# gcorso/DiffDock

Measured on AMD Instinct MI355X. Metric: poses/sec (20 steps x 40 samples, DiffDock-L score model), higher is better.
Workload: dtype f32

## Files before the change

diffdock_amd/csrc/api.cpp:

```cpp
#include <cstdlib>
#include <cstring>

#include "model.h"

using namespace ddmi;

struct ddmi_model { Model m; };

static thread_local std::string g_err;

template <class F> static int guard(F&& f) {
  try { f(); return DDMI_OK; }
  catch (const Error& e) { g_err = e.what(); return e.code; }
  catch (const std::exception& e) { g_err = e.what(); return DDMI_ERR_ARG; }
}

Routes ddmi::resolve_routes(const ddmi_config& cfg, int n_cus) {
  static const struct { const char* name; int32_t ddmi_exec_options::*field; int max; } ranges[] = {
      {"streams", &ddmi_exec_options::streams, 1}, {"dense_rows", &ddmi_exec_options::dense_rows, 2},
      {"shared_tiles", &ddmi_exec_options::shared_tiles, 2}, {"packed_granules", &ddmi_exec_options::packed_granules, 1},
      {"merged_granule", &ddmi_exec_options::merged_granule, 1}, {"pre_reduce", &ddmi_exec_options::pre_reduce, 1},
      {"hidden_mm", &ddmi_exec_options::hidden_mm, 1}, {"fc1_batch", &ddmi_exec_options::fc1_batch, 1},
      {"tile_split", &ddmi_exec_options::tile_split, 8}, {"tile_split_small", &ddmi_exec_options::tile_split_small, 8},
      {"hidden_grid", &ddmi_exec_options::hidden_grid, 1 << 20}, {"tp_apply", &ddmi_exec_options::tp_apply, 3},
// ... 178 lines not shown
    DDMI_REQUIRE(h && lig_pos && tr && rot, DDMI_ERR_ARG, "null argument");
    DDMI_CHECK_HIP(hipSetDevice(h->m.device));
    modify_conformer(h->m, lig_pos, tr, rot, tor, (hipStream_t)s);
  });
}

int ddmi_sample(ddmi_model* h, float* lig_pos, const ddmi_sample_cfg* cfg, ddmi_stream s) {
  return guard([&] {
    DDMI_REQUIRE(h && lig_pos && cfg, DDMI_ERR_ARG, "null argument");
    DDMI_CHECK_HIP(hipSetDevice(h->m.device));
    sample(h->m, lig_pos, *cfg, (hipStream_t)s);
  });
}

int ddmi_set_sample_record(ddmi_model* h, const ddmi_sample_record* r) {
  return guard([&] {
    DDMI_REQUIRE(h, DDMI_ERR_ARG, "null model");
    set_sample_record(h->m, r);
  });
}

int ddmi_perturb(ddmi_model* h, float* tr, float* rot, float* tor, const ddmi_sample_cfg* cfg, int step, ddmi_stream s) {
  return guard([&] {
    DDMI_REQUIRE(h && tr && rot && cfg, DDMI_ERR_ARG, "null argument");
    DDMI_CHECK_HIP(hipSetDevice(h->m.device));
    perturb(h->m, tr, rot, tor, *cfg, step, (hipStream_t)s);
  });
}

int ddmi_debug_shape(ddmi_model* h, const char* name, int64_t shape[4], int* ndim, int* is_int) {
  return guard([&] {
    DDMI_REQUIRE(h && name, DDMI_ERR_ARG, "null argument");
    auto it = h->m.debug.find(name);
    DDMI_REQUIRE(it != h->m.debug.end(), DDMI_ERR_KEY, std::string("unknown debug buffer: ") + name);
    *ndim = (int)it->second.shape.size();
    for (int d = 0; d < *ndim && d < 4; ++d) shape[d] = it->second.shape[d];
    *is_int = it->second.is_int;
  });
}

int ddmi_debug_read(ddmi_model* h, const char* name, void* dst, size_t bytes, ddmi_stream s) {
  return guard([&] {
    DDMI_REQUIRE(h && name && dst, DDMI_ERR_ARG, "null argument");
    auto it = h->m.debug.find(name);
    DDMI_REQUIRE(it != h->m.debug.end(), DDMI_ERR_KEY, std::string("unknown debug buffer: ") + name);
    size_t n = 4;
    for (auto d : it->second.shape) n *= (size_t)d;
    DDMI_REQUIRE(bytes <= n, DDMI_ERR_ARG, "read past the end of the buffer");
    DDMI_CHECK_HIP(hipStreamSynchronize((hipStream_t)s));
    DDMI_CHECK_HIP(hipMemcpy(dst, it->second.ptr, bytes, hipMemcpyDeviceToHost));
  });
}

int ddmi_wigner_3j(int l1, int l2, int l3, double* out) {
  return guard([&] {
    DDMI_REQUIRE(out && l1 >= 0 && l2 >= 0 && l3 >= std::abs(l1 - l2) && l3 <= l1 + l2, DDMI_ERR_ARG, "bad l");
    auto w = wigner_3j(l1, l2, l3);
    std::memcpy(out, w.data(), w.size() * sizeof(double));
  });
}

int ddmi_debug_philox(const uint32_t* counters, const uint32_t* keys, int n, uint32_t* host_out) {
  return guard([&] {
    DDMI_REQUIRE(counters && keys && host_out && n > 0, DDMI_ERR_ARG, "null argument");
    struct Buf {
      unsigned* p = nullptr;
      explicit Buf(size_t bytes) { DDMI_CHECK_HIP(hipMalloc(reinterpret_cast<void**>(&p), bytes)); }
      ~Buf() { if (p) (void)hipFree(p); }
    };
    Buf c((size_t)n * 16), k((size_t)n * 8), o((size_t)n * 16);
    hipStream_t st = nullptr;
    DDMI_CHECK_HIP(hipStreamCreateWithFlags(&st, hipStreamNonBlocking));
    struct StreamGuard { hipStream_t s; ~StreamGuard() { (void)hipStreamDestroy(s); } } sg{st};
    DDMI_CHECK_HIP(hipMemcpyAsync(c.p, counters, (size_t)n * 16, hipMemcpyHostToDevice, st));
    DDMI_CHECK_HIP(hipMemcpyAsync(k.p, keys, (size_t)n * 8, hipMemcpyHostToDevice, st));
    launch_debug_philox(c.p, k.p, n, o.p, st);
    DDMI_CHECK_HIP(hipMemcpyAsync(host_out, o.p, (size_t)n * 16, hipMemcpyDeviceToHost, st));
    DDMI_CHECK_HIP(hipStreamSynchronize(st));
// ... 32 lines not shown
```

diffdock_amd/csrc/conv_layers.cpp:

```cpp
#include <cmath>
#include <cstdio>
#include <numeric>
#include <string>

#include "cx.h"

namespace ddmi {
namespace {

long tiles_of(const RunGroup& q) {
  const long gn = std::max(1, q.gcount);
  return std::max(1L, gn * (((long)q.ea_rows / gn + 31) / 32) / 16);
}
constexpr long CHIP_TILES = 256;
bool chip_filling(long tiles) { return tiles >= CHIP_TILES; }

bool vn_fresh(const Cx& c, const RunGroup& g) {
  const Cx::VnSet& vs = c.vn[g.vn];
  return vs.built_goff == g.goff && (vs.epoch == c.epoch || (g.static_topo && vs.epoch >= 0)) && vs.built_tgt == g.tgt && vs.built_tslot == g.tslot &&
         vs.built_arow == g.arow && vs.built_nvec == g.nvec && vs.built_ew == g.ew && vs.built_sgn == g.sgn && vs.built_tbase == g.tbase;
}
void vn_mark_built(Cx& c, const RunGroup& g) {
  Cx::VnSet& vs = c.vn[g.vn];
  vs.built_goff = g.goff; vs.epoch = c.epoch; vs.built_tgt = g.tgt; vs.built_tslot = g.tslot; vs.built_arow = g.arow;
// ... 35 lines not shown
    for (int i = 0; i < LA.n; ++i) queued = queued || built[i]->vn == g.vn;
    if (queued) continue;
    DDMI_REQUIRE(LA.n < VN_GROUPS_MAX, DDMI_ERR_CAPACITY, "more edge groups than virtual-node list slots");
    Cx::VnSet& vs = c.vn[g.vn];
    const VnPoseTiles pp = pose_tiles(c, g.vn);
    LA.g[LA.n] = VnListArgs{g.goff, g.gcount, vs.voff, vs.node, vs.e0, pp.node_batch, pp.graph_ptr, pp.n_graphs, pp.nvn_pad};
    rows[LA.n] = vn_rows_args(m, g);
    if (g.vn == 0 && c.prered) {
      prered_g = &g;
      if (m.cfg.sh_lmax <= 1) { rows[LA.n].tile_hdr = vs.tile_hdr; rows[LA.n].live = vs.live; }
    }
    built[LA.n++] = &g;
  }
  if (LA.n == 0) return;
  PhaseTimer t(m, "vn_build", gs);
  launch_vn_build_all(LA, rows, m.cfg.sh_lmax, gs);
  if (prered_g && m.cfg.sh_lmax > 1) build_tile_headers(c, *prered_g, gs);
  for (int i = 0; i < LA.n; ++i) vn_mark_built(c, *built[i]);
}
void ensure_vn(Model& m, const RunGroup& g, hipStream_t gs) {
  Cx& c = *m.cx;
  Cx::VnSet& vs = c.vn[g.vn];
  if (vn_fresh(c, g)) return;
  PhaseTimer t(m, "vn_build", gs);
  const VnPoseTiles pp = pose_tiles(c, g.vn);
  launch_vn_build(g.goff, g.gcount, vs.cnt, vs.voff, vs.node, vs.e0, vn_rows_args(m, g), gs, pp.node_batch ? &pp : nullptr);
  if (g.vn == 0 && c.prered) build_tile_headers(c, g, gs);
  vn_mark_built(c, g);
}

enum class Hidden { mm, gemm, deep };
Hidden hidden_route(const Model& m, const ConvW& L, int wg) {
  if (L.TL > 2) return Hidden::deep;
  return m.r.hidden_mm && m.ns % 16 == 0 && m.ns <= 64 && L.W1p[wg] ? Hidden::mm : Hidden::gemm;
}
int weight_group(const ConvW& L, int gi) { return std::min(gi, L.G - 1); }

struct GroupRoute { bool bf, dense_rows; };
GroupRoute group_route(const Model& m, const ConvW& L, const RunGroup& g) {
  GroupRoute r;
  r.bf = m.cfg.edge_product == 1 && !L.fgran_generic && L.maxd <= 3 && m.cfg.sh_lmax <= 1;
  r.dense_rows = m.r.dense_rows == Use::always || (m.r.dense_rows == Use::by_rule && (long)g.ea_rows >= 20L * std::max(1, g.gcount));
  return r;
}

struct GroupPlan {
  int wg = 0;
  bool side = false;
  Hidden hidden = Hidden::mm;
  GroupRoute rt{};
  bool shared = false;
  float *P = nullptr, *Q = nullptr, *rowbias = nullptr, *Hb = nullptr;
  const float* rb = nullptr;
  bool last_on_stream = false;
  int ysplit = 1;
  int hidden_grid = 0;
};
struct LayerPlan {
  enum Runner { joined, grouped, overlapped } runner = joined;
  bool forked = false;
  bool small_layer = false;
  bool mm_all = false;
  int pq_mode = 0;
  int n = 0;
  GroupPlan g[VN_GROUPS_MAX];
  int issue[VN_GROUPS_MAX] = {};
};
// ... 104 lines not shown
    p.ysplit = pick_tile_split(m, L, g, P.small_layer, is_grouped ? ys_grouped : p.last_on_stream ? r.tile_split_last : 0);
    p.hidden_grid = is_grouped ? std::max(64, (int)((long)r.hidden_grid * tiles_of(g) / std::max(1L, tiles))) : r.hidden_grid;
  }
  return P;
}

template <class F> void for_fc1_terms(const Model& m, const ConvW& L, const RunGroup& g, int wg, float* P, float* Q, float* rowbias, bool sigma, F&& fn) {
  const float* W1p = L.W1p[wg];
  if (sigma && g.sig && !g.rb_ready) fn(W1p, (const float*)nullptr, rowbias, -1, m.cx->B);
  fn(W1p + (g.swap_pq ? 2 : 1) * m.ns, (const float*)nullptr, P, g.tbase, g.tcount);
  fn(W1p + (g.swap_pq ? 1 : 2) * m.ns, (const float*)L.b1p[wg], Q, g.gbase, g.gcount);
}
void launch_fc1_terms(Model& m, const ConvW& L, const RunGroup* groups, const LayerPlan& P, int g0, int g1, const float* Xin, hipStream_t s) {
  PhaseTimer t(m, "conv_fc1_gemms", s);
  GemmBatch gb;
  for (int gi = g0; gi < g1; ++gi) {
    const RunGroup& g = groups[gi];
    const GroupPlan& p = P.g[gi];
    for_fc1_terms(m, L, g, p.wg, p.P, p.Q, p.rowbias, true, [&](const float* W, const float* bias, float* C, int base, int count) {
      GemmArgs& x = batch_add(gb, s);
      if (base < 0) { x.A = g.sig; x.lda = m.ns; } else { x.A = Xin + (size_t)base * XS; x.lda = XS; }
      x.W = W; x.ldw = L.n_edge; x.bias = bias; x.C = C; x.ldc = L.H; x.M = count; x.N = L.H; x.K = m.ns;
    });
  }
  launch_gemm_batch(gb, s);
}

EdgeHiddenArgs hidden_args(Model& m, const ConvW& L, const RunGroup& g, const GroupPlan& p) {
  Cx& c = *m.cx;
  Cx::VnSet& vs = c.vn[g.vn];
  EdgeHiddenArgs h{};
  h.nvn = vn_count(c, g);
  h.vcap = vs.vcap; h.vn_node = vs.node; h.vn_e0 = vs.e0; h.goff = g.goff; h.arow = g.arow; h.tgt = g.tgt;
  h.tbase = g.tbase; h.ea = g.ea; h.ns = m.ns; h.W1 = L.W1p[p.wg]; h.ldw = L.n_edge; h.P = p.P; h.Q = p.Q; h.rowbias = p.rb; h.ridx = g.sig_idx;
  h.H = L.H; h.NG8 = L.HKq / 8; h.Hb = p.Hb; h.bf = p.rt.bf ? 1 : 0;
  h.zero_fill = (!L.fgran_generic && p.rt.dense_rows) ? 1 : 0;
  if (m.cfg.sh_lmax <= 1) { h.vrows = vs.rows; h.vn_ne = vs.ne; }
  h.grid = p.hidden_grid;
  return h;
}
FusedConvArgs fused_args(Model& m, const ConvW& L, const RunGroup& g, int gi, const GroupPlan& p, const float* Xin) {
  Cx& c = *m.cx;
  Cx::VnSet& vs = c.vn[g.vn];
  FusedConvArgs f{};
  f.nvn = vn_count(c, g);
  f.vcap = vs.vcap; f.vn_node = vs.node; f.vrows = vs.rows; f.vn_ne = vs.ne;
  f.X = Xin; f.gbase = g.gbase; f.wpack = L.wpack[p.wg]; f.KS = L.KS; f.HK = L.HK; f.Hb = p.Hb; f.NG8 = L.HKq / 8;
  f.sh_lmax = m.cfg.sh_lmax; f.gran = L.fgran; f.cgt = L.cgt;
  f.max_nb = L.max_nb; f.maxd = L.maxd; f.msg = g.msg; f.generic = L.fgran_generic ? 1 : 0;
  f.dense = p.rt.dense_rows ? 1 : 0;
  f.bf = p.rt.bf ? 1 : 0;
  f.tile_hdr = (g.vn == 0 && c.prered) ? vs.tile_hdr : nullptr;
  f.shared = p.shared ? 1 : 0;
  f.prof_slot = gi;
  fill_granule_ranges(L, p.ysplit, f);
  return f;
}

void run_group(Model& m, const ConvW& L, const RunGroup* groups, int gi, const LayerPlan& LP, const float* Xin, hipStream_t gs) {
  Cx& c = *m.cx;
  const RunGroup& g = groups[gi];
  const GroupPlan& p = LP.g[gi];
  const int ns = m.ns, H = L.H;
  DDMI_REQUIRE(g.vn >= 0 && L.n_fgran > 0 && c.Hb, DDMI_ERR_STATE, "convolution layer without a granule list / virtual-node set");
  if (m.cfg.exec.debug & 1)
    fprintf(stderr, "ddmi route %s g%d: hidden %s granules %s\n", L.name.c_str(), gi,
            p.hidden == Hidden::mm ? "mm" : p.hidden == Hidden::deep ? "deep" : "gemm", L.fgran_generic ? "generic" : "static");
// ... 220 lines not shown
```

diffdock_amd/csrc/k_hidden.hip:

```cpp
#include <algorithm>

#include "kernels.h"
#include "fc_layout.h"

namespace ddmi {

typedef float vf4 __attribute__((ext_vector_type(4)));
__device__ __forceinline__ float4 nt_load4(const float* p) {
  const vf4 v = DDMI_NT_LOAD(reinterpret_cast<const vf4*>(p));
  return make_float4(v[0], v[1], v[2], v[3]);
}

__global__ __launch_bounds__(256) void k_edge_hidden(const int* __restrict__ nvn, const int* __restrict__ vn_node,
                                                    const int* __restrict__ vn_e0, const int* __restrict__ goff,
                                                    const int* __restrict__ arow, const int* __restrict__ tgt, int tbase,
                                                    const float* __restrict__ HE, const float* __restrict__ P,
                                                    const float* __restrict__ Q, int H, int NG8, float* __restrict__ Hb, int bf) {
  const int v = blockIdx.x;
  if (v >= *nvn) return;
  const int d = vn_node[v], e0 = vn_e0[v];
  const int ne = min(32, goff[d + 1] - e0);
  const int NGP = fc_ngp(NG8), q4 = 4 * NGP;
  for (int idx = threadIdx.x; idx < 32 * q4; idx += blockDim.x) {
    const int el = idx / q4, k = 4 * (idx - el * q4);
// ... 23 lines not shown
                                                  const float* __restrict__ HE, const float* __restrict__ P,
                                                  const float* __restrict__ Q, int H, float* __restrict__ rows) {
  const int v = blockIdx.x;
  if (v >= *nvn) return;
  const int d = vn_node[v], e0 = vn_e0[v];
  const int ne = min(32, goff[d + 1] - e0);
  for (int idx = threadIdx.x; idx < ne * H; idx += blockDim.x) {
    const int el = idx / H, k = idx - el * H, e = e0 + el;
    const int ar = arow ? arow[e] : e;
    rows[(size_t)e * H + k] = fmaxf(HE[(size_t)ar * H + k] + P[(size_t)(tgt[e] - tbase) * H + k] + Q[(size_t)d * H + k], 0.f);
  }
}
void launch_edge_rows(const int* nvn, int vcap, const int* vn_node, const int* vn_e0, const int* goff, const int* arow,
                      const int* tgt, int tbase, const float* HE, const float* P, const float* Q, int H, float* rows, hipStream_t s) {
  if (vcap <= 0) return;
  hipLaunchKernelGGL(k_edge_rows, dim3(vcap), dim3(256), 0, s, nvn, vn_node, vn_e0, goff, arow, tgt, tbase, HE, P, Q, H, rows);
  DDMI_CHECK_HIP(hipGetLastError());
}
void launch_edge_hidden(const int* nvn, int vcap, const int* vn_node, const int* vn_e0, const int* goff, const int* arow,
                        const int* tgt, int tbase, const float* HE, const float* P, const float* Q, int H, int NG8,
                        float* Hb, hipStream_t s, int bf) {
  if (vcap <= 0) return;
  hipLaunchKernelGGL(k_edge_hidden, dim3(vcap), dim3(256), 0, s, nvn, vn_node, vn_e0, goff, arow, tgt, tbase, HE, P, Q, H,
                     NG8, Hb, bf);
  DDMI_CHECK_HIP(hipGetLastError());
}

__device__ __forceinline__ float f4c(const float4& v, int i) { return i == 0 ? v.x : i == 1 ? v.y : i == 2 ? v.z : v.w; }

template <int NSQ>
__device__ __forceinline__ void eh_body(const EdgeHiddenArgs& a, const int block, const int nblocks, float* __restrict__ smem) {
  constexpr int KS = 4 * NSQ;
  constexpr int H = 48 * NSQ, NB = H / 16, NG8 = H / 8;
  constexpr int HP = H + 1;
  float* wl = smem;
  const int tid = threadIdx.x, lane = tid & 63;
  const int wave = DDMI_UNIFORM(tid >> 6);
  const int lr = lane & 15, lq = lane >> 4;
  const int nvn = *a.nvn;
  if (block * 4 >= nvn) return;
  {
    constexpr int NW = (H * 4 * KS + 255) / 256;
    float wreg[NW];
#pragma unroll
    for (int it = 0; it < NW; ++it) {
      const int idx = tid + 256 * it;
      wreg[it] = idx < H * 4 * KS ? a.W1[(size_t)(idx / (4 * KS)) * a.ldw + idx % (4 * KS)] : 0.f;
    }
#pragma unroll
    for (int it = 0; it < NW; ++it) {
      const int idx = tid + 256 * it;
      const int k = idx % (4 * KS), n = idx / (4 * KS);
      const int q = k / KS, t = k - q * KS;
      if (idx < H * 4 * KS) wl[(t * 4 + q) * HP + n] = wreg[it];
    }
  }
  __syncthreads();
  for (int v = block * 4 + wave; v < nvn; v += nblocks * 4) {
    const int d = a.vn_node[v], e0 = a.vn_e0[v];
    const int ne = a.vn_ne ? a.vn_ne[v] : min(32, a.goff[d + 1] - e0);
    float4 qv[NB];
    {
      const float* __restrict__ qrow = a.Q + (size_t)d * H + 4 * lq;
#pragma unroll
      for (int nb = 0; nb < NB; ++nb) qv[nb] = *reinterpret_cast<const float4*>(qrow + 16 * nb);
      if (a.rowbias && ne > 0) {
        const float* __restrict__ rbrow = a.rowbias + (size_t)a.ridx[a.arow ? a.arow[e0] : e0] * H + 4 * lq;
#pragma unroll
        for (int nb = 0; nb < NB; ++nb) {
          const float4 t = *reinterpret_cast<const float4*>(rbrow + 16 * nb);
          qv[nb].x += t.x; qv[nb].y += t.y; qv[nb].z += t.z; qv[nb].w += t.w;
        }
      }
    }
#pragma unroll 1
    for (int rt = 0; rt < 2; ++rt) {
      float* __restrict__ hp = a.Hb + fc_hb_off(v, rt, 0, lane, NG8 / 2);
      if (16 * rt >= ne) {
        if (!a.zero_fill) continue;
#pragma unroll
        for (int nb = 0; nb < NB; ++nb) *reinterpret_cast<float4*>(hp + (size_t)nb * 256) = make_float4(0.f, 0.f, 0.f, 0.f);
        continue;
      }
      const int el = 16 * rt + lr;
      const bool live = el < ne;
      int ar, tg;
      if (a.vrows) {
        const int2 at = *reinterpret_cast<const int2*>(a.vrows + ((size_t)v * 32 + el) * 8 + 6);
        ar = at.x; tg = at.y;
      } else {
        const int e = e0 + (live ? el : 16 * rt);
        ar = a.arow ? a.arow[e] : e;
        tg = a.tgt[e] - a.tbase;
      }
#ifdef EHV_SEQATTR
      ar = e0 + (live ? el : 16 * rt);
#endif
      const float* __restrict__ ep = a.ea + (size_t)ar * a.ns + KS * lq;
      const float* __restrict__ prow = a.P + (size_t)tg * H + 4 * lq;
      float4 ae[NSQ], pv[NB];
#pragma unroll
      for (int j = 0; j < NSQ; ++j) ae[j] = *reinterpret_cast<const float4*>(ep + 4 * j);
#pragma unroll
      for (int nb = 0; nb < NB; ++nb) pv[nb] = *reinterpret_cast<const float4*>(prow + 16 * nb);
      DDMI_SCHED_FENCE();
#pragma unroll
      for (int nb = 0; nb < NB; ++nb) {
        f32x4 acc = f32x4{qv[nb].x + pv[nb].x, qv[nb].y + pv[nb].y, qv[nb].z + pv[nb].z, qv[nb].w + pv[nb].w};
        f32x4 acc2 = f32x4{0.f, 0.f, 0.f, 0.f};
        const float* __restrict__ wp = wl + lq * HP + 16 * nb + lr;
#pragma unroll
        for (int j = 0; j < NSQ; ++j) {
          acc = __builtin_amdgcn_mfma_f32_16x16x4f32(wp[(4 * j + 0) * 4 * HP], ae[j].x, acc, 0, 0, 0);
          acc2 = __builtin_amdgcn_mfma_f32_16x16x4f32(wp[(4 * j + 1) * 4 * HP], ae[j].y, acc2, 0, 0, 0);
          acc = __builtin_amdgcn_mfma_f32_16x16x4f32(wp[(4 * j + 2) * 4 * HP], ae[j].z, acc, 0, 0, 0);
          acc2 = __builtin_amdgcn_mfma_f32_16x16x4f32(wp[(4 * j + 3) * 4 * HP], ae[j].w, acc2, 0, 0, 0);
        }
        float4 o;
        o.x = live ? fmaxf(acc[0] + acc2[0], 0.f) : 0.f; o.y = live ? fmaxf(acc[1] + acc2[1], 0.f) : 0.f;
        o.z = live ? fmaxf(acc[2] + acc2[2], 0.f) : 0.f; o.w = live ? fmaxf(acc[3] + acc2[3], 0.f) : 0.f;
        if (a.bf) { bf_split2(o.x, o.y, o.x, o.y); bf_split2(o.z, o.w, o.z, o.w); }
        *reinterpret_cast<float4*>(hp + (size_t)nb * 256) = o;
      }
    }
  }
}

template <int NSQ>
__global__ __launch_bounds__(256) void k_edge_hidden_mm(EdgeHiddenArgs a) {
  DDMI_DYN_SMEM(float, smem);
  eh_body<NSQ>(a, (int)blockIdx.x, (int)gridDim.x, smem);
}
template <int NSQ>
__global__ __launch_bounds__(256) void k_edge_hidden_mm_grouped(EdgeHiddenGroupedArgs G) {
  DDMI_DYN_SMEM(float, smem);
  const int b = (int)blockIdx.x;
  int g = 0;
#pragma unroll
  for (int i = 1; i < EH_GROUPS_MAX; ++i)
    if (i < G.n && b >= G.first[i]) g = i;
  eh_body<NSQ>(G.g[g], b - G.first[g], G.first[g + 1] - G.first[g], smem);
}

void launch_edge_hidden_mm_grouped(const EdgeHiddenGroupedArgs& G_in, hipStream_t s) {
  EdgeHiddenGroupedArgs G = G_in;
  if (G.n <= 0) return;
  if (G.n > EH_GROUPS_MAX) throw Error(DDMI_ERR_ARG, "k_edge_hidden_mm_grouped: too many edge groups in one launch");
  int blocks = 0;
  const int ns = G.g[0].ns, H = G.g[0].H;
  for (int i = 0; i < G.n; ++i) {
    const EdgeHiddenArgs& a = G.g[i];
    if (a.ns != ns || a.H != H || a.ns % 16 != 0 || a.ns > 64 || a.H != 3 * a.ns || a.NG8 * 8 != a.H)
      throw Error(DDMI_ERR_ARG, "k_edge_hidden_mm_grouped: unsupported / mixed widths");
    G.first[i] = blocks;
    blocks += a.vcap > 0 ? std::max(1, std::min(cdiv(a.vcap, 4), a.grid > 0 ? a.grid : 2048)) : 0;
  }
  G.first[G.n] = blocks;
  if (blocks <= 0) return;
  const size_t smem = (size_t)(ns * (H + 1)) * sizeof(float);
  switch (ns / 16) {
    case 1: hipLaunchKernelGGL(k_edge_hidden_mm_grouped<1>, dim3(blocks), dim3(256), smem, s, G); break;
    case 2: hipLaunchKernelGGL(k_edge_hidden_mm_grouped<2>, dim3(blocks), dim3(256), smem, s, G); break;
    case 3: hipLaunchKernelGGL(k_edge_hidden_mm_grouped<3>, dim3(blocks), dim3(256), smem, s, G); break;
    default: hipLaunchKernelGGL(k_edge_hidden_mm_grouped<4>, dim3(blocks), dim3(256), smem, s, G); break;
  }
  DDMI_CHECK_HIP(hipGetLastError());
}

void launch_edge_hidden_mm(const EdgeHiddenArgs& a, hipStream_t s) {
  if (a.vcap <= 0) return;
  if (a.ns % 16 != 0 || a.ns > 64 || a.H != 3 * a.ns || a.NG8 * 8 != a.H)
    throw Error(DDMI_ERR_ARG, "k_edge_hidden_mm: unsupported width");
  const size_t smem = (size_t)(a.ns * (a.H + 1)) * sizeof(float);
  const int grid = std::min(cdiv(a.vcap, 4), a.grid > 0 ? a.grid : 2048);
  switch (a.ns / 16) {
    case 1: hipLaunchKernelGGL(k_edge_hidden_mm<1>, dim3(grid), dim3(256), smem, s, a); break;
    case 2: hipLaunchKernelGGL(k_edge_hidden_mm<2>, dim3(grid), dim3(256), smem, s, a); break;
    case 3: hipLaunchKernelGGL(k_edge_hidden_mm<3>, dim3(grid), dim3(256), smem, s, a); break;
    default: hipLaunchKernelGGL(k_edge_hidden_mm<4>, dim3(grid), dim3(256), smem, s, a); break;
  }
  DDMI_CHECK_HIP(hipGetLastError());
}


}
```

diffdock_amd/csrc/kernels.h:

```cpp
#pragma once
#include "ddmi_common.h"

namespace ddmi {

struct GemmArgs {
  const float* A = nullptr; int lda = 0;
  const float* W = nullptr; int ldw = 0;
  const float* bias = nullptr;
  const float* rowbias = nullptr; const int* ridx = nullptr; int ldrb = 0;
  float* C = nullptr; int ldc = 0;
  int M = 0, N = 0, K = 0;
  const int* m_dev = nullptr;
  int act = 0;
};
void launch_gemm(const GemmArgs& a, hipStream_t s);
constexpr int GEMM_BATCH_MAX = 16;
struct GemmBatch { GemmArgs g[GEMM_BATCH_MAX]; int n = 0; };
void launch_gemm_batch(const GemmBatch& b, hipStream_t s);

struct ObInfo { int base, itemw, mul, o_off, dout; };
struct DevPath {
  int n_off, mul_out, din, ds, dout, s_off, c_off, o_off;
  int mul_in, i_off, w_off;
  int g_off;
// ... 15 lines not shown
  int g[FC_MAXSLOT];
  int accumulate;
  int empty;
  int shape;
  int nlive;
  int dup;
  int nslot;
  int nb;
};
struct VnRowsArgs {
  const int* nvn; const int* vn_node; const int* vn_e0; const int* goff;
  const int* arow; const float* nvec; const float* ew; const int* tslot; float sgn; int sh_lmax;
  const int* tgt; int tbase;
  int vcap; float* rows; int* vn_ne;
  int* tile_hdr = nullptr; unsigned char* live = nullptr;
};
struct VnPoseTiles { const int* node_batch; const int* graph_ptr; int n_graphs; int* nvn_pad; };
void launch_vn_build(const int* goff, int gcount, int* cnt_tmp, int* voff, int* vn_node, int* vn_e0, const VnRowsArgs& rows,
                     hipStream_t s, const VnPoseTiles* pp = nullptr);
constexpr int VN_GROUPS_MAX = 9;
struct VnListArgs { const int* goff; int gcount; int* voff; int* vn_node; int* vn_e0;
                    const int* node_batch; const int* graph_ptr; int n_graphs; int* nvn_pad; };
struct VnListsArgs { int n = 0; VnListArgs g[VN_GROUPS_MAX]; };
struct VnRowsGroupedArgs { int n = 0; int first[VN_GROUPS_MAX + 1] = {}; VnRowsArgs g[VN_GROUPS_MAX]; };
static_assert(sizeof(VnRowsGroupedArgs) <= 2048 && sizeof(VnListsArgs) <= 2048, "kernel arguments");
void launch_vn_build_all(const VnListsArgs& lists, const VnRowsArgs* rows , int sh_lmax, hipStream_t s);
constexpr int FC_TILE_HDR = 36, FC_TILE_NT = 32;
void launch_vn_tiles(const int* nvn, int vcap, const float* vrows, const int* vn_ne, int* tile_hdr, unsigned char* live, hipStream_t s);
void launch_edge_hidden(const int* nvn, int vcap, const int* vn_node, const int* vn_e0, const int* goff, const int* arow,
                        const int* tgt, int tbase, const float* HE, const float* P, const float* Q, int H, int NG8,
                        float* Hb, hipStream_t s, int bf = 0);
void launch_edge_rows(const int* nvn, int vcap, const int* vn_node, const int* vn_e0, const int* goff, const int* arow,
                      const int* tgt, int tbase, const float* HE, const float* P, const float* Q, int H, float* rows, hipStream_t s);
struct EdgeHiddenArgs {
  const int* nvn; int vcap; const int* vn_node; const int* vn_e0; const int* goff;
  const int* arow; const int* tgt; int tbase;
  const float* ea; int ns;
  const float* W1; int ldw;
  const float* P;
  const float* Q;
  const float* rowbias; const int* ridx;
  int H, NG8;
  int zero_fill;
  const float* vrows; const int* vn_ne;
  float* Hb;
  int bf;
  int grid;
};
void launch_edge_hidden_mm(const EdgeHiddenArgs& a, hipStream_t s);
constexpr int EH_GROUPS_MAX = 4;
struct EdgeHiddenGroupedArgs {
  int n = 0;
  int first[EH_GROUPS_MAX + 1] = {};
  EdgeHiddenArgs g[EH_GROUPS_MAX];
};
void launch_edge_hidden_mm_grouped(const EdgeHiddenGroupedArgs& G, hipStream_t s);

struct FusedConvArgs {
  const int* nvn; int vcap;
  const int* vn_node;
  const float* vrows; const int* vn_ne;
  const float* X; int gbase;
  const float* wpack; int KS, HK;
  const float* Hb; int NG8;
  int sh_lmax;
  const FGran* gran; int ysplit; int gsplit[9];
  const float* cgt;
  int max_nb;
  int maxd;
  int generic;
  int dense;
// ... 183 lines not shown
```

diffdock_amd/csrc/model.h:

```cpp
#pragma once
#include <map>
#include <memory>
#include <string>
#include <vector>

#include "kernels.h"
#include "o3_host.h"

namespace ddmi {

struct HostTensor {
  std::vector<float> data;
  std::vector<int64_t> shape;
  int64_t numel() const { int64_t n = 1; for (auto d : shape) n *= d; return n; }
};

class DevicePool {
 public:
  ~DevicePool();
  void* alloc_bytes(size_t n);
  template <class T> T* alloc(size_t n) { return reinterpret_cast<T*>(alloc_bytes(n * sizeof(T))); }
  template <class T> T* upload(const std::vector<T>& v) {
    T* p = alloc<T>(v.size() ? v.size() : 1);
    if (!v.empty()) DDMI_CHECK_HIP(hipMemcpy(p, v.data(), v.size() * sizeof(T), hipMemcpyHostToDevice));
    return p;
  }
  void release();
  size_t total_bytes() const { return total_; }
 private:
  std::vector<void*> blocks_;
  size_t total_ = 0;
};

struct ConvW {
  std::string name;
  int G = 1;
  bool faster = false, residual = true, has_bn = true, yform = true;
  Irreps in_irr, sh_irr, out_irr;
  TPTable table;
  int n_edge = 0, H = 0, HK = 0, D_in = 0, D_out = 0, NT = 0, sh_dim = 0, Wn = 0;
  bool depthwise = false; int Wn_dw = 0, n_lin2 = 0;
  std::vector<float*> W1, b1, W2, b2, wpack;
  int TL = 2;
  std::vector<std::vector<float*>> Wmid, bmid;
  std::vector<float*> W1p, b1p;
  int KS = 0;
  FGran* fgran = nullptr; int n_fgran = 0, HKq = 0; bool fgran_generic = false;
  float* cgt = nullptr; int max_nb = 4;
  std::vector<int> fgran_unit;
  int maxd = 1;
  DevPath* paths = nullptr; float* ctab = nullptr; CgItem* items = nullptr; int n_items = 0;
  float *bn_mean = nullptr, *bn_scale = nullptr, *bn_bias = nullptr;
};

struct Mlp2W { float *W0 = nullptr, *b0 = nullptr, *W3 = nullptr, *b3 = nullptr; int in = 0, hid = 0, out = 0; };

struct DebugEntry { const void* ptr; std::vector<int64_t> shape; bool is_int; };

enum class Use { never, by_rule, always };
struct Routes {
  bool two_streams = true;
  int layer_overlap = 0;
  Use shared_tiles = Use::by_rule;
  Use dense_rows = Use::by_rule;
  bool merged_granule = true;
  bool packed_granules = true;
  int tp_form = -1;
  bool fc1_batch = true;
  bool hidden_mm = true;
  bool pre_reduce = true;
  int tile_split = 0;
  int tile_split_small = 0;
  int tile_split_last = 0;
  bool round_split = true;
  bool round_split_small = false;
  bool list_caps = false;
  bool time_terms = false;
  int group_order = 0;
// ... 20 lines not shown
  int ns = 0, sd = 0, D = 0, Dc = 0, nf = 0, lm = 0, H = 0;
  float* lig_emb = nullptr; int* lig_emb_off = nullptr;
  Mlp2W lig_enc;
  Mlp2W lig_edge, rec_edge, rec_sigma, cross_edge, center_edge, final_edge, tr_final, rot_final;
  Mlp2W atom_edge, ar_edge, la_edge;
  float* atom_emb = nullptr; int* atom_emb_off = nullptr;
  float *conf_W[3] = {}, *conf_b[3] = {}, *conf_bn_scale[2] = {}, *conf_bn_shift[2] = {};
  float *aconf_W[3] = {}, *aconf_b[3] = {};
  float* rec_emb = nullptr; float *rec_enc_W = nullptr, *rec_enc_b = nullptr;
  float *off_lig = nullptr, *off_rec = nullptr, *off_cross = nullptr, *off_center = nullptr;
  float coeff_lig = 0, coeff_rec = 0, coeff_cross = 0, coeff_center = 0;
  std::vector<ConvW> rec_emb_layers, lig_emb_layers, conv_layers;
  ConvW final_conv, tor_conv;
  std::vector<ConvW> old_lig, old_rec, old_l2r, old_r2l;
  Mlp2W old_lig_lin, old_rec_lin;
  float *old_lm_W = nullptr, *old_lm_b = nullptr;
  float *tor_W0 = nullptr, *tor_W3 = nullptr;
  float* side_Mt = nullptr; int side_K = 0;
  float* tor_T = nullptr; int tor_ds = 0, tor_dts = 0;
  float* time_freq = nullptr;
  std::vector<float> time_freq_host;
  float *so3_table = nullptr, *torus_table = nullptr; int so3_n = 0, torus_n = 0;
  bool has_complex = false;
  hipStream_t side_stream = nullptr;
  hipEvent_t ev_fork = nullptr, ev_join = nullptr, ev_cross = nullptr, ev_terms = nullptr;
  Routes r;
  std::vector<hipEvent_t> ev_pipe;
  bool uniform_t = false;
  double crop_cutoff = 0.0;
  DevicePool cpool;
  struct Cx;
  std::shared_ptr<Cx> cx;
  std::map<std::string, DebugEntry> debug;
  bool timing = false;
  int timing_level = 0;
  struct TimedPhase { std::string name; double ms = 0; int64_t launches = 0; };
  std::vector<TimedPhase> phases;
  struct EventPair { int phase; hipEvent_t a, b; };
  std::vector<EventPair> pending;
  std::vector<hipEvent_t> free_events;
};

struct PhaseTimer {
  Model& m; hipStream_t s; int idx = -1; hipEvent_t a{}, b{};
  PhaseTimer(Model& model, const char* name, hipStream_t stream);
  ~PhaseTimer();
};
void resolve_timings(Model& m);

void build_weight_spec(Model& m);
void commit_weights(Model& m);
void set_complex(Model& m, const ddmi_complex& c, hipStream_t s);
void set_batch_layout(Model& m, const ddmi_batch_layout& l, hipStream_t s);
void forward(Model& m, const float* lig_pos, const float* t_tr, const float* t_rot, const float* t_tor, float* tr_out,
             float* rot_out, float* tor_out, hipStream_t s, float* conf_out = nullptr, float* atom_conf_out = nullptr);
void sidechain_pred(Model& m, float* out, hipStream_t s);
void modify_conformer(Model& m, float* lig_pos, const float* tr, const float* rot, const float* tor, hipStream_t s,
                      float* rec_pos = nullptr);
void set_sample_record(Model& m, const ddmi_sample_record* r);
void sample(Model& m, float* lig_pos, const ddmi_sample_cfg& sc, hipStream_t s);
void perturb(Model& m, float* tr, float* rot, float* tor, const ddmi_sample_cfg& sc, int k, hipStream_t s);

}
```

diffdock_amd/csrc/weights.cpp:

```cpp
#include <algorithm>
#include <cmath>

#include "model.h"

namespace ddmi {

static const int LIG_DIMS[16] = {119, 4, 12, 12, 8, 10, 6, 6, 2, 8, 2, 2, 2, 2, 2, 2};
static const int REC_DIMS[1] = {38};
static const int ATOM_DIMS[4] = {38, 119, 23, 38};

DevicePool::~DevicePool() { release(); }
void DevicePool::release() {
  for (void* p : blocks_) (void)hipFree(p);
  blocks_.clear();
  total_ = 0;
}
void* DevicePool::alloc_bytes(size_t n) {
  void* p = nullptr;
  const size_t bytes = round_up((long)(n ? n : 1), 256);
  DDMI_CHECK_HIP(hipMalloc(&p, bytes));
  blocks_.push_back(p);
  total_ += bytes;
  return p;
}
// ... 249 lines not shown
      DDMI_REQUIRE(c.atom_num_confidence_outputs >= 1, DDMI_ERR_ARG, "atom_num_confidence_outputs must be >= 1");
      predictor("atom_confidence_predictor", n_in, c.atom_num_confidence_outputs + ns);
      n_in = ns;
    }
    predictor("confidence_predictor", n_in, c.num_confidence_outputs + (c.affinity_prediction ? 1 : 0));
    return;
  }
  if (c.sidechain_pred) {
    int n = 0;
    for (auto& b : last_out) n += b.mul * ((b.l == 0) ? 4 : (b.l == 1) ? 2 : 0);
    S.push_back({"sidechain_predictor.weight", {n}});
  }
  readout_spec(last_out);
}

static const HostTensor& W(Model& m, const std::string& k) {
  auto it = m.host_w.find(k);
  DDMI_REQUIRE(it != m.host_w.end(), DDMI_ERR_KEY, "missing state_dict key: " + k);
  return it->second;
}
static float* up(Model& m, const std::string& k) { return m.wpool.upload(W(m, k).data); }

static Mlp2W up_mlp(Model& m, const std::string& n) {
  Mlp2W r;
  const HostTensor &w0 = W(m, n + ".0.weight"), &w3 = W(m, n + ".3.weight");
  r.in = (int)w0.shape[1]; r.hid = (int)w0.shape[0]; r.out = (int)w3.shape[0];
  r.W0 = up(m, n + ".0.weight"); r.b0 = up(m, n + ".0.bias");
  r.W3 = up(m, n + ".3.weight"); r.b3 = up(m, n + ".3.bias");
  return r;
}

static void commit_conv(Model& m, ConvW& L) {
  const int H = L.H, HK = L.HK;
  L.W1.clear(); L.b1.clear(); L.W2.clear(); L.b2.clear(); L.wpack.clear(); L.W1p.clear(); L.b1p.clear(); L.Wmid.clear(); L.bmid.clear();
  std::vector<DevPath> dp;
  std::vector<float> ctab;
  std::vector<GEntry> gmap;
  int n_off = 0;
  L.maxd = 1;
  for (auto& p : L.table.paths) {
    DevPath d{};
    d.n_off = n_off; d.mul_out = p.mul_out; d.din = p.din; d.ds = p.ds; d.dout = p.dout; d.s_off = p.s_off;
    d.c_off = (int)ctab.size(); d.o_off = p.o_off; d.mul_in = p.mul_in; d.i_off = p.i_off; d.w_off = p.w_off;
    d.g_off = (int)gmap.size();
    for (int i = 0; i < p.din; ++i)
      for (int k = 0; k < p.dout; ++k) gmap.push_back({d.c_off + i * p.ds * p.dout + k, p.s_off, p.ds, p.dout});
    for (double v : p.C) ctab.push_back((float)v);
    dp.push_back(d);
    n_off += p.din * p.mul_out;
    L.maxd = std::max(L.maxd, p.dout);
  }
  std::vector<CgItem> items;
  std::vector<ObInfo> obs;
  std::vector<int> slot_base(L.table.paths.size(), 0);
  int col = 0;
  for (int ob = 0; ob < (int)L.out_irr.size(); ++ob) {
    int pb = -1, pe = -1, wi = 0;
    for (int i = 0; i < (int)L.table.paths.size(); ++i)
      if (L.table.paths[i].out_block == ob) { if (pb < 0) pb = i; pe = i + 1; slot_base[i] = wi; wi += L.table.paths[i].din; }
    if (pb < 0) { pb = pe = 0; }
    for (int w = 0; w < L.out_irr[ob].mul; ++w) items.push_back({pb, pe, L.out_irr[ob].off, L.out_irr[ob].d(), w});
    int quads = 1;
    while (quads * 4 < wi) quads *= 2;
    col = (int)round_up(col, quads * 4);
    obs.push_back({col, quads * 4, L.out_irr[ob].mul, L.out_irr[ob].off, L.out_irr[ob].d()});
    col += L.out_irr[ob].mul * quads * 4;
  }
  if (L.yform && col != L.NT) throw Error(DDMI_ERR_ARG, "internal: column layout mismatch");
  L.paths = m.wpool.upload(dp);
  L.ctab = m.wpool.upload(ctab);
  L.items = m.wpool.upload(items);
  L.n_items = (int)items.size();
  std::vector<int> wk_off(L.table.paths.size(), 0);
  int KS = 0;
  for (size_t pi = 0; pi < L.table.paths.size(); ++pi) {
    const TPPath& p = L.table.paths[pi];
    wk_off[pi] = KS;
    KS += (int)round_up(p.mul_in, 4) * (int)round_up(p.mul_out, 16);
  }
  L.KS = KS;
  for (int g = 0; g < L.G; ++g) {
    const std::string pre = L.G == 1 ? L.name + ".fc" : L.name + ".fc." + std::to_string(g);
    L.W1.push_back(up(m, pre + ".0.weight"));
    L.b1.push_back(up(m, pre + ".0.bias"));
    {
      const HostTensor &w1 = W(m, pre + ".0.weight"), &bb = W(m, pre + ".0.bias");
      const int Hh = (int)w1.shape[0], ne = (int)w1.shape[1];
      if (Hh % 16 == 0) {
        std::vector<float> wp((size_t)Hh * ne), bp(Hh);
        for (int pos = 0; pos < Hh; ++pos) {
          const int q = pos & 15, unit = (pos & ~15) + 8 * ((q & 3) >> 1) + 2 * (q >> 2) + (q & 1);
          std::copy(w1.data.begin() + (size_t)unit * ne, w1.data.begin() + (size_t)(unit + 1) * ne, wp.begin() + (size_t)pos * ne);
          bp[pos] = bb.data[unit];
        }
        L.W1p.push_back(m.wpool.upload(wp));
        L.b1p.push_back(m.wpool.upload(bp));
      } else {
        L.W1p.push_back(nullptr);
        L.b1p.push_back(nullptr);
      }
    }
    const std::string last = pre + "." + std::to_string(3 * (L.TL - 1));
    L.Wmid.emplace_back(); L.bmid.emplace_back();
    for (int j = 1; j + 1 < L.TL; ++j) {
      L.Wmid.back().push_back(up(m, pre + "." + std::to_string(3 * j) + ".weight"));
      L.bmid.back().push_back(up(m, pre + "." + std::to_string(3 * j) + ".bias"));
    }
    const HostTensor &w2s = W(m, last + ".weight"), &b2s = W(m, last + ".bias");
    HostTensor w2x, b2x;
    if (L.depthwise) {
      const HostTensor& l2 = W(m, L.name + ".linear_2.weight");
      const std::vector<DwIns> ins = depthwise_instructions(L.in_irr, L.sh_irr, L.out_irr, nullptr, nullptr);
      w2x.shape = {L.Wn, H}; w2x.data.assign((size_t)L.Wn * H, 0.f);
      b2x.shape = {L.Wn}; b2x.data.assign((size_t)L.Wn, 0.f);
      for (auto& p : L.table.paths) {
        const DwIns* q = nullptr;
        for (auto& c_ : ins)
          if (L.in_irr[c_.i1].off == p.i_off && L.sh_irr[c_.i2].off == p.s_off && c_.io == p.out_block) q = &c_;
        DDMI_REQUIRE(q && q->mul == p.mul_in, DDMI_ERR_ARG, "depthwise layer: path without an instruction");
        for (int u = 0; u < p.mul_in; ++u)
          for (int w = 0; w < p.mul_out; ++w) {
            const float f = l2.data[(size_t)q->lin_off + (size_t)(q->row_base + u) * p.mul_out + w];
            const size_t slot = (size_t)p.w_off + (size_t)u * p.mul_out + w, src = (size_t)q->w_off + u;
            for (int k = 0; k < H; ++k) w2x.data[slot * H + k] = w2s.data[src * H + k] * f;
            b2x.data[slot] = b2s.data[src] * f;
          }
      }
    }
    const HostTensor &w2 = L.depthwise ? w2x : w2s, &b2 = L.depthwise ? b2x : b2s;
    if (!L.yform) {
      L.W2.push_back(m.wpool.upload(w2.data));
      L.b2.push_back(m.wpool.upload(b2.data));
// ... 187 lines not shown
      if (blk.l == 0 && blk.p == 1) im += blk.mul;
    }
    L.bn_mean = m.wpool.upload(mean); L.bn_scale = m.wpool.upload(scale); L.bn_bias = m.wpool.upload(bias);
  }
}

static void commit_readouts(Model& m) {
  const ddmi_config& c = m.cfg;
  m.center_edge = up_mlp(m, "center_edge_embedding");
  m.tr_final = up_mlp(m, "tr_final_layer");
  m.rot_final = up_mlp(m, "rot_final_layer");
  commit_conv(m, m.final_conv);
  if (!c.no_torsion) {
    m.final_edge = up_mlp(m, "final_edge_embedding");
    commit_conv(m, m.tor_conv);
    m.tor_W0 = up(m, "tor_final_layer.0.weight");
    m.tor_W3 = up(m, "tor_final_layer.3.weight");
    Irreps tsh;
    std::vector<double> T = full_tp_dense(sh_irreps(c.sh_lmax), make_irreps({{1, 2, 1}}), &tsh);
    std::vector<float> Tf(T.begin(), T.end());
    m.tor_T = m.wpool.upload(Tf);
    m.tor_ds = (c.sh_lmax + 1) * (c.sh_lmax + 1);
    m.tor_dts = irreps_dim(tsh);
  }
}

void commit_weights(Model& m) {
  for (auto& kv : m.spec) {
    auto it = m.host_w.find(kv.first);
    DDMI_REQUIRE(it != m.host_w.end(), DDMI_ERR_KEY, "missing state_dict key: " + kv.first);
    DDMI_REQUIRE(it->second.shape == kv.second, DDMI_ERR_KEY, "shape mismatch for " + kv.first);
  }
  m.wpool.release();
  const ddmi_config& c = m.cfg;
  {
    std::vector<float> emb;
    std::vector<int> off;
    int rows = 0;
    for (int i = 0; i < 16; ++i) {
      off.push_back(rows);
      const HostTensor& t = W(m, "lig_node_embedding.atom_embedding_list." + std::to_string(i) + ".weight");
      emb.insert(emb.end(), t.data.begin(), t.data.end());
      rows += LIG_DIMS[i];
    }
    m.lig_emb = m.wpool.upload(emb);
    m.lig_emb_off = m.wpool.upload(off);
    if (!c.old_model) {
      m.lig_enc.W0 = up(m, "lig_node_embedding.additional_features_embedder.weight");
      m.lig_enc.b0 = up(m, "lig_node_embedding.additional_features_embedder.bias");
    }
  }
  m.rec_emb = up(m, "rec_node_embedding.atom_embedding_list.0.weight");
  if (c.old_model) {
    m.old_lig_lin.W0 = up(m, "lig_node_embedding.linear.weight"); m.old_lig_lin.b0 = up(m, "lig_node_embedding.linear.bias");
    m.old_rec_lin.W0 = up(m, "rec_node_embedding.linear.weight"); m.old_rec_lin.b0 = up(m, "rec_node_embedding.linear.bias");
    if (m.lm > 0) { m.old_lm_W = up(m, "rec_node_embedding.lm_embedding_layer.weight"); m.old_lm_b = up(m, "rec_node_embedding.lm_embedding_layer.bias"); }
    m.lig_edge = up_mlp(m, "lig_edge_embedding");
    m.rec_edge = up_mlp(m, "rec_edge_embedding");
    m.cross_edge = up_mlp(m, "cross_edge_embedding");
    if (c.confidence_mode) {
      for (int i = 0; i < 3; ++i) {
        m.conf_W[i] = up(m, "confidence_predictor." + std::to_string(4 * i) + ".weight");
        m.conf_b[i] = up(m, "confidence_predictor." + std::to_string(4 * i) + ".bias");
      }
      for (int i = 0; i < 2; ++i) {
        const std::string n = "confidence_predictor." + std::to_string(4 * i + 1);
// ... 149 lines not shown
```

Baseline: 159.5.

## Prebuild padded W1 shared-memory image and software-pipeline edge hidden kernel loads

At weight-commit time, the fc1 weights are reordered on the host into the exact padded shared-memory layout the edge-hidden kernel uses. The kernel can then stage them with coalesced float4 copies instead of strided scalar gathers and index math. The per-node loop becomes a flat software pipeline: the next tile's indices, edge attributes and P/Q rows are loaded before the current tile's compute finishes, and the first tile's loads overlap the weight staging. This costs more live registers for the prefetched data and an extra device weight image per layer. It also adds a debug map for these images.

```diff
diff --git a/diffdock_amd/csrc/api.cpp b/diffdock_amd/csrc/api.cpp
--- a/diffdock_amd/csrc/api.cpp
+++ b/diffdock_amd/csrc/api.cpp
@@ -234,7 +234,10 @@
   return guard([&] {
     DDMI_REQUIRE(h && name, DDMI_ERR_ARG, "null argument");
     auto it = h->m.debug.find(name);
-    DDMI_REQUIRE(it != h->m.debug.end(), DDMI_ERR_KEY, std::string("unknown debug buffer: ") + name);
+    if (it == h->m.debug.end()) {
+      it = h->m.wdebug.find(name);
+      DDMI_REQUIRE(it != h->m.wdebug.end(), DDMI_ERR_KEY, std::string("unknown debug buffer: ") + name);
+    }
     *ndim = (int)it->second.shape.size();
     for (int d = 0; d < *ndim && d < 4; ++d) shape[d] = it->second.shape[d];
     *is_int = it->second.is_int;
@@ -245,7 +248,10 @@
   return guard([&] {
     DDMI_REQUIRE(h && name && dst, DDMI_ERR_ARG, "null argument");
     auto it = h->m.debug.find(name);
-    DDMI_REQUIRE(it != h->m.debug.end(), DDMI_ERR_KEY, std::string("unknown debug buffer: ") + name);
+    if (it == h->m.debug.end()) {
+      it = h->m.wdebug.find(name);
+      DDMI_REQUIRE(it != h->m.wdebug.end(), DDMI_ERR_KEY, std::string("unknown debug buffer: ") + name);
+    }
     size_t n = 4;
     for (auto d : it->second.shape) n *= (size_t)d;
     DDMI_REQUIRE(bytes <= n, DDMI_ERR_ARG, "read past the end of the buffer");
diff --git a/diffdock_amd/csrc/conv_layers.cpp b/diffdock_amd/csrc/conv_layers.cpp
--- a/diffdock_amd/csrc/conv_layers.cpp
+++ b/diffdock_amd/csrc/conv_layers.cpp
@@ -91,7 +91,7 @@
 enum class Hidden { mm, gemm, deep };
 Hidden hidden_route(const Model& m, const ConvW& L, int wg) {
   if (L.TL > 2) return Hidden::deep;
-  return m.r.hidden_mm && m.ns % 16 == 0 && m.ns <= 64 && L.W1p[wg] ? Hidden::mm : Hidden::gemm;
+  return m.r.hidden_mm && m.ns % 16 == 0 && m.ns <= 64 && L.W1img[wg] ? Hidden::mm : Hidden::gemm;
 }
 int weight_group(const ConvW& L, int gi) { return std::min(gi, L.G - 1); }
 
@@ -262,7 +262,7 @@
   EdgeHiddenArgs h{};
   h.nvn = vn_count(c, g);
   h.vcap = vs.vcap; h.vn_node = vs.node; h.vn_e0 = vs.e0; h.goff = g.goff; h.arow = g.arow; h.tgt = g.tgt;
-  h.tbase = g.tbase; h.ea = g.ea; h.ns = m.ns; h.W1 = L.W1p[p.wg]; h.ldw = L.n_edge; h.P = p.P; h.Q = p.Q; h.rowbias = p.rb; h.ridx = g.sig_idx;
+  h.tbase = g.tbase; h.ea = g.ea; h.ns = m.ns; h.W1img = L.W1img[p.wg]; h.P = p.P; h.Q = p.Q; h.rowbias = p.rb; h.ridx = g.sig_idx;
   h.H = L.H; h.NG8 = L.HKq / 8; h.Hb = p.Hb; h.bf = p.rt.bf ? 1 : 0;
   h.zero_fill = (!L.fgran_generic && p.rt.dense_rows) ? 1 : 0;
   if (m.cfg.sh_lmax <= 1) { h.vrows = vs.rows; h.vn_ne = vs.ne; }
diff --git a/diffdock_amd/csrc/k_hidden.hip b/diffdock_amd/csrc/k_hidden.hip
--- a/diffdock_amd/csrc/k_hidden.hip
+++ b/diffdock_amd/csrc/k_hidden.hip
@@ -79,77 +79,83 @@
 __device__ __forceinline__ void eh_body(const EdgeHiddenArgs& a, const int block, const int nblocks, float* __restrict__ smem) {
   constexpr int KS = 4 * NSQ;
   constexpr int H = 48 * NSQ, NB = H / 16, NG8 = H / 8;
-  constexpr int HP = H + 1;
+  constexpr int HP = eh_img_stride(H);
   float* wl = smem;
   const int tid = threadIdx.x, lane = tid & 63;
   const int wave = DDMI_UNIFORM(tid >> 6);
   const int lr = lane & 15, lq = lane >> 4;
   const int nvn = *a.nvn;
   if (block * 4 >= nvn) return;
+  int d = 0, e0 = 0, ne = 0, ar = 0, tg = 0;
+  float4 qv[NB], ae[NSQ], pv[NB];
+  auto tile_index = [&](int v, int rt) {
+    const int el = 16 * rt + lr;
+    if (a.vrows) {
+      const int2 at = *reinterpret_cast<const int2*>(a.vrows + ((size_t)v * 32 + el) * 8 + 6);
+      ar = at.x; tg = at.y;
+    } else {
+      const int e = e0 + (el < ne ? el : 16 * rt);
+      ar = a.arow ? a.arow[e] : e;
+      tg = a.tgt[e] - a.tbase;
+    }
+#ifdef EHV_SEQATTR
+    ar = e0 + (el < ne ? el : 16 * rt);
+#endif
+  };
+  auto tile_rows = [&]() {
+    const float* __restrict__ ep = a.ea + (size_t)ar * a.ns + KS * lq;
+    const float* __restrict__ prow = a.P + (size_t)tg * H + 4 * lq;
+#pragma unroll
+    for (int j = 0; j < NSQ; ++j) ae[j] = *reinterpret_cast<const float4*>(ep + 4 * j);
+#pragma unroll
+    for (int nb = 0; nb < NB; ++nb) pv[nb] = *reinterpret_cast<const float4*>(prow + 16 * nb);
+  };
+  auto node_header = [&](int v) {
+    d = a.vn_node[v]; e0 = a.vn_e0[v];
+    ne = a.vn_ne ? a.vn_ne[v] : min(32, a.goff[d + 1] - e0);
+  };
+  auto node_q = [&]() {
+    const float* __restrict__ qrow = a.Q + (size_t)d * H + 4 * lq;
+#pragma unroll
+    for (int nb = 0; nb < NB; ++nb) qv[nb] = *reinterpret_cast<const float4*>(qrow + 16 * nb);
+    if (a.rowbias && ne > 0) {
+      const float* __restrict__ rbrow = a.rowbias + (size_t)a.ridx[a.arow ? a.arow[e0] : e0] * H + 4 * lq;
+#pragma unroll
+      for (int nb = 0; nb < NB; ++nb) {
+        const float4 t = *reinterpret_cast<const float4*>(rbrow + 16 * nb);
+        qv[nb].x += t.x; qv[nb].y += t.y; qv[nb].z += t.z; qv[nb].w += t.w;
+      }
+    }
+  };
+  int v = block * 4 + wave;
   {
-    constexpr int NW = (H * 4 * KS + 255) / 256;
-    float wreg[NW];
-#pragma unroll
-    for (int it = 0; it < NW; ++it) {
-      const int idx = tid + 256 * it;
-      wreg[it] = idx < H * 4 * KS ? a.W1[(size_t)(idx / (4 * KS)) * a.ldw + idx % (4 * KS)] : 0.f;
-    }
-#pragma unroll
-    for (int it = 0; it < NW; ++it) {
-      const int idx = tid + 256 * it;
-      const int k = idx % (4 * KS), n = idx / (4 * KS);
-      const int q = k / KS, t = k - q * KS;
-      if (idx < H * 4 * KS) wl[(t * 4 + q) * HP + n] = wreg[it];
-    }
+    constexpr int NI = KS * HP, NW = (NI + 255) / 256;
+    if (v < nvn) { node_header(v); if (ne > 0) tile_index(v, 0); }
+#ifndef EHV_NOSTAGE
+    float4 wreg[NW];
+    const float4* __restrict__ wi = reinterpret_cast<const float4*>(a.W1img);
+#pragma unroll
+    for (int it = 0; it < NW; ++it)
+      wreg[it] = (256 * (it + 1) <= NI || tid + 256 * it < NI) ? wi[tid + 256 * it] : make_float4(0.f, 0.f, 0.f, 0.f);
+    DDMI_SCHED_FENCE();
+#pragma unroll
+    for (int it = 0; it < NW; ++it)
+      if (256 * (it + 1) <= NI || tid + 256 * it < NI) reinterpret_cast<float4*>(wl)[tid + 256 * it] = wreg[it];
+    DDMI_SCHED_FENCE();
+#endif
+    if (v < nvn) { node_q(); if (ne > 0) tile_rows(); }
   }
   __syncthreads();
-  for (int v = block * 4 + wave; v < nvn; v += nblocks * 4) {
-    const int d = a.vn_node[v], e0 = a.vn_e0[v];
-    const int ne = a.vn_ne ? a.vn_ne[v] : min(32, a.goff[d + 1] - e0);
-    float4 qv[NB];
-    {
-      const float* __restrict__ qrow = a.Q + (size_t)d * H + 4 * lq;
-#pragma unroll
-      for (int nb = 0; nb < NB; ++nb) qv[nb] = *reinterpret_cast<const float4*>(qrow + 16 * nb);
-      if (a.rowbias && ne > 0) {
-        const float* __restrict__ rbrow = a.rowbias + (size_t)a.ridx[a.arow ? a.arow[e0] : e0] * H + 4 * lq;
-#pragma unroll
-        for (int nb = 0; nb < NB; ++nb) {
-          const float4 t = *reinterpret_cast<const float4*>(rbrow + 16 * nb);
-          qv[nb].x += t.x; qv[nb].y += t.y; qv[nb].z += t.z; qv[nb].w += t.w;
-        }
-      }
-    }
-#pragma unroll 1
-    for (int rt = 0; rt < 2; ++rt) {
-      float* __restrict__ hp = a.Hb + fc_hb_off(v, rt, 0, lane, NG8 / 2);
-      if (16 * rt >= ne) {
-        if (!a.zero_fill) continue;
+  int rt = 0;
+  while (v < nvn) {
+    float* __restrict__ hp = a.Hb + fc_hb_off(v, rt, 0, lane, NG8 / 2);
+    if (16 * rt >= ne) {
+      if (a.zero_fill) {
 #pragma unroll
         for (int nb = 0; nb < NB; ++nb) *reinterpret_cast<float4*>(hp + (size_t)nb * 256) = make_float4(0.f, 0.f, 0.f, 0.f);
-        continue;
-      }
-      const int el = 16 * rt + lr;
-      const bool live = el < ne;
-      int ar, tg;
-      if (a.vrows) {
-        const int2 at = *reinterpret_cast<const int2*>(a.vrows + ((size_t)v * 32 + el) * 8 + 6);
-        ar = at.x; tg = at.y;
-      } else {
-        const int e = e0 + (live ? el : 16 * rt);
-        ar = a.arow ? a.arow[e] : e;
-        tg = a.tgt[e] - a.tbase;
-      }
-#ifdef EHV_SEQATTR
-      ar = e0 + (live ? el : 16 * rt);
-#endif
-      const float* __restrict__ ep = a.ea + (size_t)ar * a.ns + KS * lq;
-      const float* __restrict__ prow = a.P + (size_t)tg * H + 4 * lq;
-      float4 ae[NSQ], pv[NB];
-#pragma unroll
-      for (int j = 0; j < NSQ; ++j) ae[j] = *reinterpret_cast<const float4*>(ep + 4 * j);
-#pragma unroll
-      for (int nb = 0; nb < NB; ++nb) pv[nb] = *reinterpret_cast<const float4*>(prow + 16 * nb);
+      }
+    } else {
+      const bool live = 16 * rt + lr < ne;
       DDMI_SCHED_FENCE();
 #pragma unroll
       for (int nb = 0; nb < NB; ++nb) {
@@ -170,6 +176,15 @@
         *reinterpret_cast<float4*>(hp + (size_t)nb * 256) = o;
       }
     }
+    DDMI_SCHED_FENCE();
+    if (rt == 0) {
+      rt = 1;
+    } else {
+      rt = 0;
+      v += nblocks * 4;
+      if (v < nvn) { node_header(v); node_q(); }
+    }
+    if (v < nvn && 16 * rt < ne) { tile_index(v, rt); tile_rows(); }
   }
 }
 
@@ -197,14 +212,14 @@
   const int ns = G.g[0].ns, H = G.g[0].H;
   for (int i = 0; i < G.n; ++i) {
     const EdgeHiddenArgs& a = G.g[i];
-    if (a.ns != ns || a.H != H || a.ns % 16 != 0 || a.ns > 64 || a.H != 3 * a.ns || a.NG8 * 8 != a.H)
+    if (a.ns != ns || a.H != H || a.ns % 16 != 0 || a.ns > 64 || a.H != 3 * a.ns || a.NG8 * 8 != a.H || !a.W1img)
       throw Error(DDMI_ERR_ARG, "k_edge_hidden_mm_grouped: unsupported / mixed widths");
     G.first[i] = blocks;
     blocks += a.vcap > 0 ? std::max(1, std::min(cdiv(a.vcap, 4), a.grid > 0 ? a.grid : 2048)) : 0;
   }
   G.first[G.n] = blocks;
   if (blocks <= 0) return;
-  const size_t smem = (size_t)(ns * (H + 1)) * sizeof(float);
+  const size_t smem = (size_t)(ns * eh_img_stride(H)) * sizeof(float);
   switch (ns / 16) {
     case 1: hipLaunchKernelGGL(k_edge_hidden_mm_grouped<1>, dim3(blocks), dim3(256), smem, s, G); break;
     case 2: hipLaunchKernelGGL(k_edge_hidden_mm_grouped<2>, dim3(blocks), dim3(256), smem, s, G); break;
@@ -216,9 +231,9 @@
 
 void launch_edge_hidden_mm(const EdgeHiddenArgs& a, hipStream_t s) {
   if (a.vcap <= 0) return;
-  if (a.ns % 16 != 0 || a.ns > 64 || a.H != 3 * a.ns || a.NG8 * 8 != a.H)
+  if (a.ns % 16 != 0 || a.ns > 64 || a.H != 3 * a.ns || a.NG8 * 8 != a.H || !a.W1img)
     throw Error(DDMI_ERR_ARG, "k_edge_hidden_mm: unsupported width");
-  const size_t smem = (size_t)(a.ns * (a.H + 1)) * sizeof(float);
+  const size_t smem = (size_t)(a.ns * eh_img_stride(a.H)) * sizeof(float);
   const int grid = std::min(cdiv(a.vcap, 4), a.grid > 0 ? a.grid : 2048);
   switch (a.ns / 16) {
     case 1: hipLaunchKernelGGL(k_edge_hidden_mm<1>, dim3(grid), dim3(256), smem, s, a); break;
diff --git a/diffdock_amd/csrc/kernels.h b/diffdock_amd/csrc/kernels.h
--- a/diffdock_amd/csrc/kernels.h
+++ b/diffdock_amd/csrc/kernels.h
@@ -71,11 +71,12 @@
                         float* Hb, hipStream_t s, int bf = 0);
 void launch_edge_rows(const int* nvn, int vcap, const int* vn_node, const int* vn_e0, const int* goff, const int* arow,
                       const int* tgt, int tbase, const float* HE, const float* P, const float* Q, int H, float* rows, hipStream_t s);
+constexpr int eh_img_stride(int H) { return H + 1; }
 struct EdgeHiddenArgs {
   const int* nvn; int vcap; const int* vn_node; const int* vn_e0; const int* goff;
   const int* arow; const int* tgt; int tbase;
   const float* ea; int ns;
-  const float* W1; int ldw;
+  const float* W1img;
   const float* P;
   const float* Q;
   const float* rowbias; const int* ridx;
diff --git a/diffdock_amd/csrc/model.h b/diffdock_amd/csrc/model.h
--- a/diffdock_amd/csrc/model.h
+++ b/diffdock_amd/csrc/model.h
@@ -44,6 +44,7 @@
   int TL = 2;
   std::vector<std::vector<float*>> Wmid, bmid;
   std::vector<float*> W1p, b1p;
+  std::vector<float*> W1img;
   int KS = 0;
   FGran* fgran = nullptr; int n_fgran = 0, HKq = 0; bool fgran_generic = false;
   float* cgt = nullptr; int max_nb = 4;
@@ -130,6 +131,7 @@
   struct Cx;
   std::shared_ptr<Cx> cx;
   std::map<std::string, DebugEntry> debug;
+  std::map<std::string, DebugEntry> wdebug;
   bool timing = false;
   int timing_level = 0;
   struct TimedPhase { std::string name; double ms = 0; int64_t launches = 0; };
diff --git a/diffdock_amd/csrc/weights.cpp b/diffdock_amd/csrc/weights.cpp
--- a/diffdock_amd/csrc/weights.cpp
+++ b/diffdock_amd/csrc/weights.cpp
@@ -305,7 +305,7 @@
 
 static void commit_conv(Model& m, ConvW& L) {
   const int H = L.H, HK = L.HK;
-  L.W1.clear(); L.b1.clear(); L.W2.clear(); L.b2.clear(); L.wpack.clear(); L.W1p.clear(); L.b1p.clear(); L.Wmid.clear(); L.bmid.clear();
+  L.W1.clear(); L.b1.clear(); L.W2.clear(); L.b2.clear(); L.wpack.clear(); L.W1p.clear(); L.b1p.clear(); L.W1img.clear(); L.Wmid.clear(); L.bmid.clear();
   std::vector<DevPath> dp;
   std::vector<float> ctab;
   std::vector<GEntry> gmap;
@@ -368,9 +368,22 @@
         }
         L.W1p.push_back(m.wpool.upload(wp));
         L.b1p.push_back(m.wpool.upload(bp));
+        const int ns = m.ns;
+        if (ns % 16 == 0 && ns <= 64 && Hh == 3 * ns && ne >= ns) {
+          const int HP = eh_img_stride(Hh), KSq = ns / 4;
+          std::vector<float> img((size_t)ns * HP, 0.f);
+          for (int t = 0; t < KSq; ++t)
+            for (int q = 0; q < 4; ++q)
+              for (int n = 0; n < Hh; ++n) img[(size_t)(t * 4 + q) * HP + n] = wp[(size_t)n * ne + q * KSq + t];
+          L.W1img.push_back(m.wpool.upload(img));
+          m.wdebug["w1img." + L.name + "." + std::to_string(g)] = DebugEntry{L.W1img.back(), {(int64_t)ns, (int64_t)HP}, false};
+        } else {
+          L.W1img.push_back(nullptr);
+        }
       } else {
         L.W1p.push_back(nullptr);
         L.b1p.push_back(nullptr);
+        L.W1img.push_back(nullptr);
       }
     }
     const std::string last = pre + "." + std::to_string(3 * (L.TL - 1));
@@ -624,6 +637,7 @@
     DDMI_REQUIRE(it->second.shape == kv.second, DDMI_ERR_KEY, "shape mismatch for " + kv.first);
   }
   m.wpool.release();
+  m.wdebug.clear();
   const ddmi_config& c = m.cfg;
   {
     std::vector<float> emb;
```

New measurement: 160.5 (median of 6 runs). About the same (+0.6%).
